# manasakani/DeviceKMC

Measured on AMD Instinct MI355X. Metric: KMC steps/sec, higher is better.
Workload: dtype f64

## Files before the change

### devicekmc_amd/csrc/common.h

```cpp
#pragma once
#include <hip/hip_runtime.h>
#include <stdint.h>
#include <stdio.h>
#include <string.h>
#include <math.h>
#include "../../include/devicekmc_hip.h"
#include "../../include/devicekmc_hip_debug.h"

enum { DEFECT = 0, OXYGEN_DEFECT = 1, VACANCY = 2, O_EL = 3, Hf_EL = 4, Ni_EL = 5, Ti_EL = 6, Pt_EL = 7, N_EL = 8, NULL_ELEMENT = 9 };
enum { EV_GEN = 0, EV_REC = 1, EV_VDIFF = 2, EV_IDIFF = 3, EV_NULL = 4 };

#define DKMC_KB 8.617333262e-5
#define DKMC_Q 1.60217663e-19
#define DKMC_HBAR 1.054571817e-34
#define DKMC_MAX_LAYERS 5
#define WAVE 64

struct MetalSet { int n; const int *e; };

__device__ __forceinline__ bool is_metal(int el, const MetalSet &ms)
{
    bool r = false;
    for (int t = 0; t < ms.n; ++t) r |= (ms.e[t] == el);
    return r;
// ... 152 lines not shown
    int x_poly1_degree = 0;
    int x_poly_form_used = 0, x_poly_products = 0;
    int x_slab_poly = 0;
    int x_aux_warm = 0;
    int x_items_kc = 0;
    int x_apply_form = 0;
    int x_tile_f32 = 1;
    double x_tile_drop = 0.0;
    int x_tile_drop_unit = 0;
    int x_tile_drop_auto = 1;
    long long x_tile_drop_gate = 0;
    double x_tile_drop_used = 0.0;
    int xtl_census_form = 1;
    int x_static_tiles = 2;
    int x_static_gate = 0;
    int x_static_nM = -1;
    int x_static_verify = 0;
    int x_tile_f32_fail_once = 0;
    int x_nmul_form = 1;
    int x_nmul_lane_bytes = 16;
    int x_nmul_window = 2;
    int x_nmul_window_cap = 76 * 1024;
    int x_nmul_window_block = 320;
    int x_block = 16;
    int x_format = 1;
    int current_map = 0;
    int x_iter_hint = 0;
    int event_temperature = 0;
    int event_census = 0;
    int event_census_valid = 0;
    double event_census_info[16] = {0};
    dkmc_stats stats{};
    char err[512] = {0};
    int err_code = 0;
    double E_gen[DKMC_MAX_LAYERS] = {0}, E_rec[DKMC_MAX_LAYERS] = {0}, E_Vdiff[DKMC_MAX_LAYERS] = {0}, E_Odiff[DKMC_MAX_LAYERS] = {0};
    int num_layers = 0;
    static const int NBUF = 184;
    void *buf[NBUF] = {nullptr};
    size_t bufsz[NBUF] = {0};
};

constexpr int X_STATIC_GATE = 32768;
static inline int x_static_rule(int ns, int gate_override) { return ns >= (gate_override > 0 ? gate_override : X_STATIC_GATE) ? 1 : 0; }
Engine &eng();
int dkmc_fail(int code, const char *what, const char *file, int line);
void *scratch(int slot, size_t bytes);
// ... 66 lines not shown
```

### devicekmc_amd/csrc/engine.hip

```cpp
#include "common.h"
#include <stdlib.h>

int events_upload_layers();
void xstate_reset(const void *key);

static Engine g_engine;
Engine &eng() { return g_engine; }

int dkmc_fail(int code, const char *what, const char *file, int line)
{
    Engine &e = eng();
    snprintf(e.err, sizeof(e.err), "%s (%s:%d)", what, file, line);
    e.err_code = code ? code : -1;
    fprintf(stderr, "devicekmc_hip: %s\n", e.err);
    return e.err_code;
}

void *scratch(int slot, size_t bytes)
{
    Engine &e = eng();
    if (bytes == 0) bytes = 16;
    if (e.bufsz[slot] < bytes) {
        if (e.buf[slot]) { (void)hipStreamSynchronize(e.stream); (void)hipFree(e.buf[slot]); }
        size_t want = bytes + bytes / 8 + 256;
// ... 64 lines not shown
void dkmc_set_x_tile_drop_auto(int on) { eng().x_tile_drop_auto = on ? 1 : 0; }
int dkmc_get_x_tile_drop_auto(void) { return eng().x_tile_drop_auto; }
void dkmc_set_x_tile_drop_auto_subblocks(long long gate) { eng().x_tile_drop_gate = gate > 0 ? gate : 0; }
double dkmc_get_x_tile_drop_used(void) { return eng().x_tile_drop_used; }
void dkmc_debug_fail_true_residual_once(void) { eng().x_tile_f32_fail_once = 1; }
void dkmc_set_x_static_tiles(int mode) { eng().x_static_tiles = (mode == 0 || mode == 1) ? mode : 2; }
int dkmc_get_x_static_tiles(void) { return eng().x_static_tiles; }
int dkmc_debug_x_static_verify(int on) { const int was = eng().x_static_verify; eng().x_static_verify = on ? 1 : 0; return was; }
void dkmc_debug_set_x_static_gate(int members) { eng().x_static_gate = members > 0 ? members : 0; }
int dkmc_x_static_rule(int members) { return x_static_rule(members, eng().x_static_gate); }
int dkmc_x_static_strips(int n_metals) { return n_metals > 0 ? n_metals / 256 : 0; }
void dkmc_set_x_nmul_form(int form) { eng().x_nmul_form = form == 0 ? 0 : 1; }
int dkmc_get_x_nmul_form(void) { return eng().x_nmul_form; }
void dkmc_set_x_nmul_lane_bytes(int bytes) { eng().x_nmul_lane_bytes = bytes == 8 ? 8 : 16; }
int dkmc_get_x_nmul_lane_bytes(void) { return eng().x_nmul_lane_bytes; }
void dkmc_set_x_nmul_window(int mode) { eng().x_nmul_window = (mode == 0 || mode == 1) ? mode : 2; }
int dkmc_get_x_nmul_window(void) { return eng().x_nmul_window; }
void dkmc_debug_set_x_nmul_window(int cap_bytes, int block_rows)
{
    Engine &e = eng();
    e.x_nmul_window_cap = cap_bytes < 0 ? 76 * 1024 : (cap_bytes > 76 * 1024 ? 76 * 1024 : cap_bytes);
    e.x_nmul_window_block = (block_rows >= 16 && block_rows <= 1024 && block_rows % 16 == 0) ? block_rows : 320;
}
void dkmc_set_x_slab(int on) { eng().x_slab = on ? 1 : 0; }
int dkmc_get_x_slab(void) { return eng().x_slab; }
void dkmc_set_x_slab_poly(int on) { eng().x_slab_poly = on ? 1 : 0; }
int dkmc_get_x_slab_poly(void) { return eng().x_slab_poly; }
void dkmc_set_x_block(int s) { eng().x_block = s < 1 ? 1 : (s > 16 ? 16 : s); }
int dkmc_get_x_block(void) { return eng().x_block; }
void dkmc_set_x_aux(int mode) { eng().x_aux = mode < 0 ? 0 : (mode > 3 ? 2 : mode); }
int dkmc_get_x_aux(void) { return eng().x_aux; }
void dkmc_set_k_blocked(int on) { eng().k_blocked = on ? 1 : 0; }
int dkmc_get_k_blocked(void) { return eng().k_blocked; }
void dkmc_set_k_blocked_large(int on) { eng().k_blocked_large = on ? 1 : 0; }
int dkmc_get_k_blocked_large(void) { return eng().k_blocked_large; }
void dkmc_set_k_window_word_bytes(int bytes) { eng().k_window_word_bytes = bytes == 2 ? 2 : 4; }
int dkmc_get_k_window_word_bytes(void) { return eng().k_window_word_bytes; }
void dkmc_set_cb_edge_domain(int atoms_only) { eng().cb_edge_domain = atoms_only ? 1 : 0; }

int dkmc_get_gpu_info(char *gpu_string, int capacity, int dev)
{
    hipDeviceProp_t prop;
    HIPCHK(hipSetDevice(dev));
    HIPCHK(hipGetDeviceProperties(&prop, dev));
    snprintf(gpu_string, capacity, "%s", prop.name);
    return 0;
// ... 117 lines not shown
```

### devicekmc_amd/csrc/nwin_plan.h

```cpp
#pragma once

#ifdef __HIPCC__
#define NWIN_HD __host__ __device__
#else
#define NWIN_HD
#endif

#define NWIN_ROW_BYTES 128
#define NWIN_CAP_BYTES (76 * 1024)
#define NWIN_BLOCK 320
#define NWIN_BLOCK_MAX 1024

struct NwinWindow { int lo, n; };

NWIN_HD inline int nwin_cap_rows(int cap_bytes) { return cap_bytes > 0 ? cap_bytes / NWIN_ROW_BYTES : 0; }
NWIN_HD inline int nwin_block_rows(int B) { return (B >= 16 && B <= NWIN_BLOCK_MAX && B % 16 == 0) ? B : NWIN_BLOCK; }
NWIN_HD inline int nwin_blocks(int m, int B) { return m > 0 ? (m + B - 1) / B : 0; }
NWIN_HD inline NwinWindow nwin_window(int m, int B, int cap_rows, int b)
{
    const int r0 = b * B, r1 = r0 + B < m ? r0 + B : m;
    if (cap_rows <= 0 || r0 >= m) return {0, 0};
    if (cap_rows < B) return {r0, r1 - r0 < cap_rows ? r1 - r0 : cap_rows};
    const int h = (cap_rows - B) / 2, lo = r0 - h > 0 ? r0 - h : 0, hi = r1 + h < m ? r1 + h : m;
    return {lo, hi - lo};
}
NWIN_HD inline int nwin_code(int c, NwinWindow W) { const int rel = c - W.lo; return (unsigned)rel < (unsigned)W.n ? rel : ~c; }
NWIN_HD inline int nwin_lds_bytes(int m, int B, int cap_rows)
{
    int n = B + 2 * ((cap_rows - B) / 2);
    if (cap_rows < B) n = cap_rows;
    if (n > m) n = m;
    return (n > 1 ? n : 1) * NWIN_ROW_BYTES;
}
NWIN_HD inline bool nwin_use(int mode, int m, int gate_rows) { return mode == 1 || (mode == 2 && m >= gate_rows); }
```

### devicekmc_amd/csrc/xtb_precond.h

```cpp
#pragma once
#include "nwin_plan.h"
__device__ __forceinline__ int xtb_xcd_block(int nb, int b) { const int xq = nb >> 3, xr = nb & 7, xc = b & 7; return xc * xq + min(xc, xr) + (b >> 3); }
template <int U> __device__ __forceinline__ int xn_bc(int x) { return __builtin_amdgcn_update_dpp(0, x, 0x150 + U, 0xf, 0xf, false); }
template <int J> __device__ __forceinline__ int xn_bc2(int x) { return __builtin_amdgcn_update_dpp(__builtin_amdgcn_update_dpp(0, x, 0x150 + 2 * J, 0xf, 0x3, false), x, 0x151 + 2 * J, 0xf, 0xc, false); }
struct XnEntry { int c, wlo, whi; };
__device__ __forceinline__ XnEntry xn_entry(int c, double w) { return {c, __double2loint(w), __double2hiint(w)}; }
template <int U> __device__ __forceinline__ double xn_w(XnEntry e) { return __hiloint2double(xn_bc<U>(e.whi), xn_bc<U>(e.wlo)); }
template <int J> __device__ __forceinline__ double xn_w2(XnEntry e) { return __hiloint2double(xn_bc2<J>(e.whi), xn_bc2<J>(e.wlo)); }
template <bool MASKED, int U> __device__ __forceinline__ double xn_gather(const double *panel, int v, int c)
{
    const int cu = xn_bc<U>(c);
    return (!MASKED || cu >= 0) ? *reinterpret_cast<const double *>(reinterpret_cast<const char *>(panel) + ((unsigned)cu * (unsigned)(XB_SP * 8) + (unsigned)(v * 8))) : 0.0;
}
struct XnX4 { double x0, x1, x2, x3; };
template <bool MASKED, int U> __device__ __forceinline__ XnX4 xn_gather4(const double *panel, int v, int c)
{
    return {xn_gather<MASKED, U>(panel, v, c), xn_gather<MASKED, U + 1>(panel, v, c), xn_gather<MASKED, U + 2>(panel, v, c), xn_gather<MASKED, U + 3>(panel, v, c)};
}
template <int J> __device__ __forceinline__ double2 xn_gather2(const double *panel, int v8, int c)
{ return *reinterpret_cast<const double2 *>(reinterpret_cast<const char *>(panel) + ((unsigned)xn_bc2<J>(c) * (unsigned)(XB_SP * 8) + (unsigned)(v8 * 16))); }
struct XnSums { double s0, s1, s2, s3; };
template <int U> __device__ __forceinline__ XnSums xn_acc4(XnEntry e, XnX4 x, XnSums s)
{
    s.s0 += xn_w<U>(e) * x.x0; s.s1 += xn_w<U + 1>(e) * x.x1; s.s2 += xn_w<U + 2>(e) * x.x2; s.s3 += xn_w<U + 3>(e) * x.x3; return s;
// ... 19 lines not shown
    const int v = threadIdx.x & 15, g = threadIdx.x >> 4;
    const int li = xtb_xcd_block((int)gridDim.x, (int)blockIdx.x) * 16 + g;
    const bool ok = li < m;
    const int row = LIST ? (ok ? rowlist[li] : 0) : li;
    const bool atom = ok && row >= 2;
    const xrp_t p0 = atom ? rp[row] : 0, p1 = atom ? rp[row + 1] : 0;
    const double scr = ok ? sc[row] : 0.0;
    const double av = ok ? add[(size_t)row * XB_SP + v] : 0.0;
    XnSums s = {0.0, 0.0, 0.0, 0.0};
    for (xrp_t base = p0; base < p1; base += 64) {
        int cm[4]; double wm[4];
#pragma unroll
        for (int bq = 0; bq < 4; ++bq) { const xrp_t pe = base + 16 * bq + v; int c = pe < p1 ? ci[pe] : -1; if (c < 2 || c == row) c = -1; cm[bq] = c; wm[bq] = c >= 0 ? val[pe] : 0.0; }
#pragma unroll
        for (int bq = 0; bq < 4; ++bq) wm[bq] = cm[bq] >= 0 ? wm[bq] * sc[cm[bq]] : 0.0;
#pragma unroll
        for (int bq = 0; bq < 4; ++bq) {
            if (base + 16 * bq >= p1) break;
            s = xn_batch16(in, v, xn_entry(cm[bq], wm[bq]), s);
        }
    }
    if (ok) out[(size_t)row * XB_SP + v] = xn_result(ca, av, cb, scr, s);
}
__global__ void k_xtb_npack_width(int m, const xrp_t *__restrict__ rp, int *__restrict__ cnt, const int *__restrict__ rowlist = nullptr)
{
    const int q = blockIdx.x * blockDim.x + threadIdx.x;
    if (q >= (m + 3) / 4) return;
    int w = 0;
    for (int r = 0; r < 4; ++r) {
        const int li = 4 * q + r; if (li >= m) continue;
        const int row = rowlist ? rowlist[li] : li;
        if (row >= 2) w = max(w, (int)(rp[row + 1] - rp[row]));
    }
    cnt[q] = 4 * w;
}
__global__ __launch_bounds__(256) void k_xtb_npack(int m, const xrp_t *__restrict__ rp, const int *__restrict__ ci, const double *__restrict__ val,
                                                   const double *__restrict__ sc, const long long *__restrict__ off, int *__restrict__ pcol, double *__restrict__ pw,
                                                   const int *__restrict__ rowlist = nullptr)
{
    const int q = blockIdx.x * 4 + (threadIdx.x >> 6), lane = threadIdx.x & 63;
    if (q >= (m + 3) / 4) return;
    const long long o0 = off[q], n = off[q + 1] - o0;
    for (long long i = lane; i < n; i += 64) {
        const int r = (int)(i & 3), k = (int)(i >> 2), li = 4 * q + r;
        const int row = rowlist ? rowlist[li < m ? li : m - 1] : li;
        const bool atom = row >= 2 && li < m;
        const xrp_t p0 = atom ? rp[row] : 0, len = atom ? rp[row + 1] - p0 : 0;
        int c = k < len ? ci[p0 + k] : -1;
        double w = 0.0;
// ... 131 lines not shown
            const int t = R.w - k0; const XnEntry e = xn_entry(nwin_code(n.c, W), n.w);
            if (t > 16) n = xn_slot(R, k0 + 16 + v);
            double2 x[4];
            x[0] = xn_operand2<0>(in, win, v8, e.c); x[1] = xn_operand2<1>(in, win, v8, e.c);
            if (t > 4) { x[2] = xn_operand2<2>(in, win, v8, e.c); x[3] = xn_operand2<3>(in, win, v8, e.c); }
            s = xn_acc2<0>(e, x[0], x[1], s);
            if (t > 4) s = xn_acc2<2>(e, x[2], x[3], s);
            if (t > 8) {
                x[0] = xn_operand2<4>(in, win, v8, e.c); x[1] = xn_operand2<5>(in, win, v8, e.c);
                if (t > 12) { x[2] = xn_operand2<6>(in, win, v8, e.c); x[3] = xn_operand2<7>(in, win, v8, e.c); }
                s = xn_acc2<4>(e, x[0], x[1], s);
                if (t > 12) s = xn_acc2<6>(e, x[2], x[3], s);
            }
        }
        if (QSF && wr) av = *reinterpret_cast<const double2 *>(add + (size_t)R.row * XB_SP + 2 * v8);
        const double tA0 = xor_lane<8>(s.A0), tA1 = xor_lane<8>(s.A1), tB0 = xor_lane<8>(s.B0), tB1 = xor_lane<8>(s.B1);
        if (wr) {
            const double o0 = xn_result(ca, av.x, cb, scr, {s.A0, tA0, s.B0, tB0}), o1 = xn_result(ca, av.y, cb, scr, {s.A1, tA1, s.B1, tB1});
            *reinterpret_cast<double2 *>(out + (size_t)R.row * XB_SP + 2 * v8) = make_double2(o0, o1);
            if (QSF) { const int sr = nsrank[R.row]; if (sr >= 0) { QS[xtb_qs_pos(sr, 2 * v8)] = scr * o0; QS[xtb_qs_pos(sr, 2 * v8 + 1)] = scr * o1; } }
        }
    }
}
__global__ void k_xtb_qs_from(int m, const double *__restrict__ V, const double *__restrict__ sc, const int *__restrict__ nsrank, double *__restrict__ QS, const XCtrl *ctrl)
{
    const int i = blockIdx.x * blockDim.x + threadIdx.x;
    if (i >= m * XB_SP || ctrl->done) return;
    const int row = i >> 4, v = i & 15;
    const int sr = nsrank[row];
    if (sr >= 0) QS[xtb_qs_pos(sr, v)] = sc[row] * V[i];
}
__global__ void k_xtb_pre_resid(int m, const double *__restrict__ T, const double *__restrict__ b, double *__restrict__ W)
{
    const int i = blockIdx.x * blockDim.x + threadIdx.x;
    if (i >= m * XB_SP) return;
    W[i] = (i & 15) == 0 ? T[i] - b[i >> 4] : 0.0;
}
__global__ void k_xtb_pre_col0(int m, const double *__restrict__ y, double *__restrict__ W)
{
    const int i = blockIdx.x * blockDim.x + threadIdx.x;
    if (i >= m * XB_SP) return;
    W[i] = (i & 15) == 0 ? y[i >> 4] : 0.0;
}
__global__ void k_xtb_pre_add(int m, const double *__restrict__ Z, double *__restrict__ y)
{
    const int i = blockIdx.x * blockDim.x + threadIdx.x;
// ... 3 lines not shown
__device__ __forceinline__ double xtb_tree256(double a)
{
    __shared__ double red[256];
    red[threadIdx.x] = a;
    __syncthreads();
    for (int o = 128; o > 0; o >>= 1) { if ((int)threadIdx.x < o) red[threadIdx.x] += red[threadIdx.x + o]; __syncthreads(); }
    return red[0];
}
__global__ __launch_bounds__(256) void k_xtb_pre_rr_part(int m, const double *__restrict__ T, const double *__restrict__ b, double *__restrict__ part)
{
    double a = 0.0;
    for (int i = blockIdx.x * 256 + threadIdx.x; i < m; i += gridDim.x * 256) { const double d = T[(size_t)i * XB_SP] - b[i]; a += d * d; }
    a = xtb_tree256(a);
    if (threadIdx.x == 0) part[blockIdx.x] = a;
}
__global__ __launch_bounds__(256) void k_xtb_pre_rr(int np, const double *__restrict__ part, double *__restrict__ out)
{
    double a = 0.0;
    for (int i = threadIdx.x; i < np; i += 256) a += part[i];
    a = xtb_tree256(a);
    if (threadIdx.x == 0) out[0] = a;
}

struct XbNPack { const long long *off; const int *col; const double *w; int lane_bytes; int win_B, win_rows; };
static const int xb_nwin_rows = 450000;
template <class Alloc>
static int xtb_npack(const XtbArgs &A, int n, const int *rowlist, Alloc alloc, long long pad, XbNPack *np)
{
    Engine &e = eng(); hipStream_t st = e.stream;
    const int nsl = (n + 3) / 4;
    int *cnt = (int *)alloc(S_XTB_NPACK_CNT, (size_t)nsl * 4);
    long long *off = (long long *)alloc(S_XTB_NPACK_OFF, (size_t)(nsl + 1) * 8);
    if (!cnt || !off) return e.err_code;
    hipLaunchKernelGGL(k_xtb_npack_width, dim3((nsl + 255) / 256), dim3(256), 0, st, n, A.rp, cnt, rowlist);
    if (int rc = dkmc_exclusive_scan_i32_i64(cnt, off, nsl, off + nsl)) return rc;
    long long nslot = 0;
    HIPCHK(hipMemcpyAsync(&nslot, off + nsl, sizeof(long long), hipMemcpyDeviceToHost, st));
    HIPCHK(hipStreamSynchronize(st));
    int *col = (int *)alloc(S_XTB_NPACK_COL, (size_t)(nslot + pad) * 4);
    double *w = (double *)alloc(S_XTB_NPACK_W, (size_t)(nslot + pad) * 8);
    if (!col || !w) return e.err_code;
    hipLaunchKernelGGL(k_xtb_npack, dim3((nsl + 3) / 4), dim3(256), 0, st, n, A.rp, A.ci, A.val, A.sc, (const long long *)off, col, w, rowlist);
    KCHK();
    np->off = off; np->col = col; np->w = w; np->lane_bytes = e.x_nmul_lane_bytes;
    const bool win = !rowlist && np->lane_bytes == 16 && nwin_use(e.x_nmul_window, n, xb_nwin_rows);
    np->win_B = win ? nwin_block_rows(e.x_nmul_window_block) : 0;
    np->win_rows = win ? nwin_cap_rows(std::min(std::max(e.x_nmul_window_cap, 0), NWIN_CAP_BYTES)) : 0;
    return 0;
}
struct XbNRank { int n; const int *rowlist; const XbNPack *np; double *QS; const XCtrl *ctrl; };
template <bool LIST>
static void xtb_nstep(hipStream_t st, const XtbArgs &A, const XbNRank &R, const double *in, const double *add, double ca, double cb, double *out, bool qsf)
{
    const dim3 g((R.n + 15) / 16), b(XT_NT);
    if (!R.np) { hipLaunchKernelGGL(k_xtb_nmul<LIST>, g, b, 0, st, R.n, A.rp, A.ci, A.val, A.sc, in, add, ca, cb, out, R.ctrl, R.rowlist); return; }
    if (!LIST && R.np->win_B > 0) {
        const int B = R.np->win_B, lds = nwin_lds_bytes(R.n, B, R.np->win_rows);
        const auto kw = qsf ? k_xtb_nmulw<true> : k_xtb_nmulw<false>;
        static bool big_lds = false;
        if (!big_lds) {
            (void)hipFuncSetAttribute((const void *)k_xtb_nmulw<true>, hipFuncAttributeMaxDynamicSharedMemorySize, NWIN_CAP_BYTES);
            (void)hipFuncSetAttribute((const void *)k_xtb_nmulw<false>, hipFuncAttributeMaxDynamicSharedMemorySize, NWIN_CAP_BYTES);
            big_lds = true;
        }
        hipLaunchKernelGGL(kw, dim3(nwin_blocks(R.n, B)), dim3(XN_WIN_NT), lds, st, R.n, R.np->off, R.np->col, R.np->w, A.sc, in, add, ca, cb, out, R.ctrl,
                           qsf ? A.nsrank : (const int *)nullptr, qsf ? R.QS : (double *)nullptr, B, R.np->win_rows);
        return;
    }
    const bool b16 = R.np->lane_bytes == 16;
    const auto k = qsf ? (b16 ? k_xtb_nmulp16<true, LIST> : k_xtb_nmulp<true, LIST>) : (b16 ? k_xtb_nmulp16<false, LIST> : k_xtb_nmulp<false, LIST>);
    hipLaunchKernelGGL(k, g, b, 0, st, R.n, R.np->off, R.np->col, R.np->w, A.sc, in, add, ca, cb, out, R.ctrl, qsf ? A.nsrank : (const int *)nullptr,
                       qsf ? R.QS : (double *)nullptr, R.rowlist);
}
template <class Pn, class Pre, class Ranks>
static int xtb_applyL(hipStream_t st, const XtbArgs &A, int pd, const double *pc, Pn src, Pn dst, Pn w1, Pn w2, bool qs, Pre pre, Ranks ranks)
{
    Pn in = src;
    for (int i = 0; i < pd; ++i) {
// ... 77 lines not shown
}

extern "C" int dkmc_xtb_poly_coeffs(int degree, double *pc)
{
    if (degree < 1 || degree > XB_MAXPOLY || !pc) return dkmc_fail(13, "xtb_poly_coeffs: degree outside 1 ... 16", __FILE__, __LINE__);
    xtb_poly_coeffs(degree, pc);
    return 0;
}
extern "C" int dkmc_xtb_poly1_coeffs(int n, double *pc, double *qmin)
{
    if (n < 1 || n > XB_MAXPOLY1 || !pc) return dkmc_fail(13, "xtb_poly1_coeffs: degree outside 1 ... 20", __FILE__, __LINE__);
    xtb_poly1_coeffs(n, pc, qmin);
    return 0;
}
extern "C" int dkmc_xtb_poly_rule(int m) { return xtb_poly_rule(m, eng().x_poly_rows); }
__global__ void k_xtb_test_qs_decode(int ns, const double *__restrict__ QS, double *__restrict__ out)
{
    const int i = blockIdx.x * blockDim.x + threadIdx.x;
    if (i < ns * XB_SP) out[i] = QS[xtb_qs_pos(i >> 4, i & 15)];
}
static void *xtb_test_alloc(int slot, size_t bytes)
{
    return scratch(slot == S_XTB_NPACK_CNT ? S_XTB_TEST_NPCNT : slot == S_XTB_NPACK_OFF ? S_XTB_TEST_NPOFF : slot == S_XTB_NPACK_COL ? S_XTB_TEST_NPCOL : S_XTB_TEST_NPW, bytes);
}
static int xtb_test_qs_out(hipStream_t st, int ns, const double *QS, double *qs)
{
    double *dq = (double *)scratch(S_XTB_TEST_ADD, (size_t)ns * XB_SP * 8);
    if (!dq) return eng().err_code;
    hipLaunchKernelGGL(k_xtb_test_qs_decode, dim3((unsigned)(((size_t)ns * XB_SP + 255) / 256)), dim3(256), 0, st, ns, QS, dq);
    KCHK();
    HIPCHK(hipMemcpyAsync(qs, dq, (size_t)ns * XB_SP * 8, hipMemcpyDeviceToHost, st));
    return 0;
}
extern "C" int dkmc_xtb_test_nstep(int m, const long long *rp, const int *ci, const double *val, const double *sc, const double *in, const double *add,
                                   double ca, double cb, int form, const int *rowlist, int nlist, const int *nsrank, int ns, double *out, double *qs)
{
    Engine &e = eng(); hipStream_t st = e.stream;
    if (m < 1 || !rp || !sc || !in || !add || !out || (form != 0 && form != 1)) return dkmc_fail(13, "xtb_test_nstep: bad arguments", __FILE__, __LINE__);
    const long long nnz = rp[m];
    if (rp[0] != 0 || nnz < 0 || nnz > 0x7fffffffll || (nnz > 0 && (!ci || !val))) return dkmc_fail(13, "xtb_test_nstep: bad row pointers", __FILE__, __LINE__);
    for (int i = 0; i < m; ++i) if (rp[i + 1] < rp[i]) return dkmc_fail(13, "xtb_test_nstep: bad row pointers", __FILE__, __LINE__);
    for (long long p = 0; p < nnz; ++p) if (ci[p] < 0 || ci[p] >= m) return dkmc_fail(13, "xtb_test_nstep: column outside the rows", __FILE__, __LINE__);
    if (rowlist) {
        if (nlist < 1 || nlist > m) return dkmc_fail(13, "xtb_test_nstep: bad row list", __FILE__, __LINE__);
        for (int i = 0; i < nlist; ++i) if (rowlist[i] < 0 || rowlist[i] >= m) return dkmc_fail(13, "xtb_test_nstep: bad row list", __FILE__, __LINE__);
    }
// ... 112 lines not shown
```

### devicekmc_amd/lib.py

```python
import ctypes as C
import os

_HERE = os.path.dirname(os.path.abspath(__file__))
LIB_PATH = os.path.join(_HERE, "libdevicekmc_hip.so")

c_int_p = C.POINTER(C.c_int)
c_dbl_p = C.POINTER(C.c_double)
vp = C.c_void_p


class dkmc_gpubuf(C.Structure):
    _PTRS = ["site_charge", "site_power", "site_potential_boundary", "site_potential_charge", "site_temperature",
             "site_CB_edge", "T_bg", "atom_power", "atom_CB_edge", "atom_virtual_potentials", "atom_charge",
             "site_element", "atom_element", "site_x", "site_y", "site_z", "atom_x", "atom_y", "atom_z",
             "metal_types", "sigma", "k", "lattice", "freq", "neigh_idx", "site_layer",
             "Device_row_ptr_d", "Device_col_indices_d", "contact_left_row_ptr", "contact_left_col_indices",
             "contact_right_row_ptr", "contact_right_col_indices"]
    _INTS = ["Device_nnz", "contact_left_nnz", "contact_right_nnz", "num_metal_types_", "N_", "nn_", "N_atom_"]
    _fields_ = [(n, vp) for n in _PTRS] + [(n, C.c_int) for n in _INTS]


class dkmc_stats(C.Structure):
    _fields_ = [("cg_iters_K", C.c_int), ("cg_iters_CB", C.c_int), ("cg_iters_X", C.c_int),
                ("cg_rr_K", C.c_double), ("cg_rr_CB", C.c_double), ("cg_rr_X", C.c_double),
# ... 57 lines not shown
    "dkmc_get_x_tile_drop_auto": (_I, []),
    "dkmc_get_x_tile_drop_used": (_D, []),
    "dkmc_get_x_tile_live_info": (_I, [C.POINTER(C.c_longlong), c_dbl_p]),
    "dkmc_xt_get_live": (_I, [_D, vp, vp]),
    "dkmc_xt_get_live_masks": (_I, [_D, vp]),
    "dkmc_debug_fail_true_residual_once": (None, []),
    "dkmc_set_x_static_tiles": (None, [_I]),
    "dkmc_get_x_static_tiles": (_I, []),
    "dkmc_get_x_static_info": (_I, [C.POINTER(C.c_longlong)]),
    "dkmc_debug_x_static_verify": (_I, [_I]),
    "dkmc_debug_get_x_static_verify": (_I, [C.POINTER(C.c_longlong)]),
    "dkmc_x_static_strips": (_I, [_I]),
    "dkmc_x_static_rule": (_I, [_I]),
    "dkmc_debug_set_x_static_gate": (None, [_I]),
    "dkmc_xt_get_srow": (_I, [c_int_p, vp]),
    "dkmc_xt_get_diag": (_I, [vp]),
    "dkmc_set_x_nmul_form": (None, [_I]),
    "dkmc_get_x_nmul_form": (_I, []),
    "dkmc_set_x_nmul_lane_bytes": (None, [_I]),
    "dkmc_get_x_nmul_lane_bytes": (_I, []),
    "dkmc_set_x_nmul_window": (None, [_I]),
    "dkmc_get_x_nmul_window": (_I, []),
    "dkmc_debug_set_x_nmul_window": (None, [_I, _I]),
    "dkmc_set_x_apply_form": (None, [_I]),
    "dkmc_get_x_apply_form": (_I, []),
    "dkmc_set_x_slab": (None, [_I]),
    "dkmc_get_x_slab": (_I, []),
    "dkmc_set_x_slab_poly": (None, [_I]),
    "dkmc_get_x_slab_poly": (_I, []),
    "dkmc_set_x_aux_warm": (None, [_I]),
    "dkmc_get_x_aux_warm": (_I, []),
    "dkmc_set_x_aux": (None, [_I]),
    "dkmc_get_x_aux": (_I, []),
    "dkmc_set_k_blocked": (None, [_I]),
    "dkmc_get_k_blocked": (_I, []),
    "dkmc_set_k_blocked_large": (None, [_I]),
    "dkmc_get_k_blocked_large": (_I, []),
    "dkmc_set_k_window_word_bytes": (None, [_I]),
    "dkmc_get_k_window_word_bytes": (_I, []),
    "dkmc_kcg_form_info": (_I, [C.POINTER(dkmc_gpubuf), C.POINTER(C.c_longlong)]),
    "dkmc_kcg_form_words": (_I, [C.POINTER(dkmc_gpubuf), C.POINTER(C.c_longlong)]),
    "dkmc_debug_kbw_halfword_pos": (_I, [_I, _I]),
    "dkmc_debug_kbw_segment_cap": (None, [_I]),
    "dkmc_set_pair_cutoff": (None, [_D]),
    "dkmc_reset_pair_sum_cache": (None, []),
    "dkmc_set_pair_form": (None, [_I]),
# ... 162 lines not shown
```

### include/devicekmc_hip.h

```cpp
#ifndef DEVICEKMC_HIP_H
#define DEVICEKMC_HIP_H

#ifdef __cplusplus
extern "C" {
#endif

#ifndef DKMC_ELEMENT_T
#define DKMC_ELEMENT_T int
#endif
typedef struct dkmc_gpubuf {
    int *site_charge;
    double *site_power, *site_potential_boundary, *site_potential_charge, *site_temperature;
    double *site_CB_edge;
    double *T_bg;
    double *atom_power;
    double *atom_CB_edge;
    double *atom_virtual_potentials;
    int *atom_charge;
    DKMC_ELEMENT_T *site_element;
    DKMC_ELEMENT_T *atom_element;
    double *site_x, *site_y, *site_z;
    double *atom_x, *atom_y, *atom_z;
    DKMC_ELEMENT_T *metal_types;
    double *sigma, *k, *lattice, *freq;
// ... 66 lines not shown
int dkmc_get_x_poly_auto(void);
void dkmc_set_x_poly_form(int form);
int dkmc_get_x_poly_form(void);
int dkmc_get_x_poly_form_used(void);
int dkmc_get_x_poly_products(void);
void dkmc_set_x_nmul_form(int form);
int dkmc_get_x_nmul_form(void);
void dkmc_set_x_tile_f32(int mode);
int dkmc_get_x_tile_f32(void);
void dkmc_set_x_tile_drop(double theta);
double dkmc_get_x_tile_drop(void);
void dkmc_set_x_tile_drop_unit(int unit);
int dkmc_get_x_tile_drop_unit(void);
void dkmc_set_x_tile_drop_auto(int on);
int dkmc_get_x_tile_drop_auto(void);
double dkmc_get_x_tile_drop_used(void);
void dkmc_set_x_static_tiles(int mode);
int dkmc_get_x_static_tiles(void);
int dkmc_get_x_static_info(long long *info8);
void dkmc_set_x_nmul_lane_bytes(int bytes);
int dkmc_get_x_nmul_lane_bytes(void);
void dkmc_set_x_nmul_window(int mode);
int dkmc_get_x_nmul_window(void);
void dkmc_set_x_slab(int on);
int dkmc_get_x_slab(void);
void dkmc_set_x_slab_poly(int on);
int dkmc_get_x_slab_poly(void);
void dkmc_set_k_slab(int on);
int dkmc_get_k_slab(void);
void dkmc_set_x_aux(int mode);
int dkmc_get_x_aux(void);
void dkmc_set_x_aux_warm(int on);
int dkmc_get_x_aux_warm(void);
void dkmc_set_k_blocked(int on);
int dkmc_get_k_blocked(void);
void dkmc_set_k_blocked_large(int on);
int dkmc_get_k_blocked_large(void);
void dkmc_set_k_window_word_bytes(int bytes);
int dkmc_get_k_window_word_bytes(void);
void dkmc_set_current_warm_start(int mode);
int dkmc_get_current_warm_start(void);
int dkmc_get_current_warm_vector(const dkmc_gpubuf *buf, double *h_out, int capacity, int *n_out);
int dkmc_set_current_warm_vector(const dkmc_gpubuf *buf, const double *h_in, int n);
int dkmc_get_current_warm_aux(const dkmc_gpubuf *buf, double *h_out, long long capacity, long long *n_out);
int dkmc_set_current_warm_aux(const dkmc_gpubuf *buf, const double *h_in, long long n);
void dkmc_set_profiling(int on);
// ... 168 lines not shown
```

### include/devicekmc_hip_debug.h

```cpp
#ifndef DEVICEKMC_HIP_DEBUG_H
#define DEVICEKMC_HIP_DEBUG_H
#include "devicekmc_hip.h"
#ifdef __cplusplus
extern "C" {
#endif

int dkmc_xt_time_share(int nranks, int rank, int reps, double *apply_us, double *side_us , int *items_out, long long *subblocks_out);
int dkmc_xt_check_shares(int nranks, double *max_abs_diff, double *max_abs, long long *subblocks_sum, long long *items_sum, int *items_total);
int dkmc_xtb_check_product(int width, double *max_abs_diff, double *max_abs);
int dkmc_xtb_poly_coeffs(int degree, double *pc);
int dkmc_xtb_poly_rule(int m);
void dkmc_set_x_poly_auto_rows(int n0, int n1);
int dkmc_xtb_test_nstep(int m, const long long *rp, const int *ci, const double *val, const double *sc, const double *in, const double *add,
                        double ca, double cb, int form, const int *rowlist, int nlist, const int *nsrank, int ns, double *out, double *qs);
int dkmc_xtb_check_poly(int degree, int form, const double *in, double *out, double *qs);
void dkmc_debug_set_x_nmul_window(int cap_bytes, int block_rows);
int dkmc_xtb_time_poly(int degree, int reps, double *us);
typedef struct dkmc_xtb_ctrl { double rr[2]; int done_local, sharded; int done; int iters; int abort_local, aborted; int pad[2]; int xchg_timeout, pad2; } dkmc_xtb_ctrl;
int dkmc_xtb_test_gram(int m, const double *P, const double *T, const double *R, const int *nsrank, int ns, int ng, int done_word, double *gfin,
                       dkmc_xtb_ctrl *ctrl_out);
int dkmc_xtb_test_small(int it, int s, int nrg, const double *gblocks, double tol2, const dkmc_xtb_ctrl *ctrl_in, double *mats, dkmc_xtb_ctrl *ctrl_out);
int dkmc_xtb_test_step(int m, int it, const double *mats, int done_word, double *y0, double *R, double *P, const double *T, const double *sc,
                       const int *nsrank, int ns, const int *rowlist, int nlist, double *Ypanel, double *qs);
int dkmc_xtb_poly1_coeffs(int n, double *pc, double *qmin);
void dkmc_debug_set_x_poly1_degree(int n);
int dkmc_xtb_test_gram1(int m, const double *const *panels, int ng, int done_word, double *gfin);
int dkmc_xtb_test_step1(int m, int it, const double *mats, int done_word, double *y0, double *const *panels, const double *sc, const int *nsrank, int ns,
                        double *qs);
int dkmc_xtb_time_apply(int width, int variant, int reps, double *us);
int dkmc_xt_tile_census(long long *hist);
void dkmc_set_x_items(int kc);
void dkmc_debug_fail_true_residual_once(void);
int dkmc_xtb_tile_product(int width, int stored_bytes, double *out);
int dkmc_xt_get_tiles(long long *ntiles, long long *nsub, int *tiles4, double *tval);
int dkmc_xtb_time_apply_stored(int width, int stored_bytes, int reps, double *us);
int dkmc_get_x_tile_live_info(long long *info8, double *ms2);
int dkmc_debug_xtl_census_form(int form);
long long dkmc_debug_xtl_census_reread(void);
double dkmc_xtl_drop_rule(long long stored_subblocks);
// ... 47 lines not shown
```

Before: 5.266.

## Add class-coded packed neighbor multiply that drops the per-slot weight array

```diff
diff --git a/devicekmc_amd/csrc/common.h b/devicekmc_amd/csrc/common.h
--- a/devicekmc_amd/csrc/common.h
+++ b/devicekmc_amd/csrc/common.h
@@ -198,6 +198,11 @@
     int x_nmul_window = 2;
     int x_nmul_window_cap = 76 * 1024;
     int x_nmul_window_block = 320;
+    int x_nmul_coded = 2;
+    int x_nmul_coded_cap = 76 * 1024;
+    int x_nmul_coded_block = 320;
+    int x_nmul_coded_halo = 126;
+    int x_nmul_coded_list = 0;
     int x_block = 16;
     int x_format = 1;
     int current_map = 0;
diff --git a/devicekmc_amd/csrc/engine.hip b/devicekmc_amd/csrc/engine.hip
--- a/devicekmc_amd/csrc/engine.hip
+++ b/devicekmc_amd/csrc/engine.hip
@@ -110,6 +110,16 @@
     e.x_nmul_window_cap = cap_bytes < 0 ? 76 * 1024 : (cap_bytes > 76 * 1024 ? 76 * 1024 : cap_bytes);
     e.x_nmul_window_block = (block_rows >= 16 && block_rows <= 1024 && block_rows % 16 == 0) ? block_rows : 320;
 }
+void dkmc_set_x_nmul_coded(int mode) { eng().x_nmul_coded = (mode == 0 || mode == 1) ? mode : 2; }
+int dkmc_get_x_nmul_coded(void) { return eng().x_nmul_coded; }
+void dkmc_debug_set_x_nmul_lists(int cap_bytes, int block_rows, int halo_rows, int list_rows)
+{
+    Engine &e = eng();
+    e.x_nmul_coded_cap = cap_bytes < 0 ? 76 * 1024 : (cap_bytes > 76 * 1024 ? 76 * 1024 : cap_bytes);
+    e.x_nmul_coded_block = (block_rows >= 16 && block_rows <= 1024 && block_rows % 16 == 0) ? block_rows : 320;
+    e.x_nmul_coded_halo = (halo_rows >= 0 && halo_rows <= 4096) ? halo_rows : 126;
+    e.x_nmul_coded_list = 0; (void)list_rows;
+}
 void dkmc_set_x_slab(int on) { eng().x_slab = on ? 1 : 0; }
 int dkmc_get_x_slab(void) { return eng().x_slab; }
 void dkmc_set_x_slab_poly(int on) { eng().x_slab_poly = on ? 1 : 0; }
diff --git a/devicekmc_amd/csrc/nwin_plan.h b/devicekmc_amd/csrc/nwin_plan.h
--- a/devicekmc_amd/csrc/nwin_plan.h
+++ b/devicekmc_amd/csrc/nwin_plan.h
@@ -33,3 +33,25 @@
     return (n > 1 ? n : 1) * NWIN_ROW_BYTES;
 }
 NWIN_HD inline bool nwin_use(int mode, int m, int gate_rows) { return mode == 1 || (mode == 2 && m >= gate_rows); }
+
+#define NWINC_ROW_BYTES (NWIN_ROW_BYTES + 8)
+#define NWINC_CLS_SHIFT 30
+#define NWINC_COL_MASK 0x3fffffffu
+#define NWINC_MAX_ROWS (1 << 28)
+#define NWINC_BLOCK 320
+#define NWINC_HALO 126
+#define NWINC_HALO_MAX 4096
+
+NWIN_HD inline unsigned nwinc_word(int c, int cls) { return (unsigned)c | ((unsigned)cls << NWINC_CLS_SHIFT); }
+NWIN_HD inline int nwinc_col(unsigned w) { return (int)(w & NWINC_COL_MASK); }
+NWIN_HD inline int nwinc_cls(unsigned w) { return (int)(w >> NWINC_CLS_SHIFT); }
+NWIN_HD inline int nwinc_block_rows(int B) { return (B >= 16 && B <= NWIN_BLOCK_MAX && B % 16 == 0) ? B : NWINC_BLOCK; }
+NWIN_HD inline int nwinc_halo_rows(int h) { return (h >= 0 && h <= NWINC_HALO_MAX) ? h : NWINC_HALO; }
+NWIN_HD inline int nwinc_rows(int cap_bytes, int B, int halo_rows)
+{
+    const int n = cap_bytes > 0 ? cap_bytes / NWINC_ROW_BYTES : 0;
+    return n > B + 2 * halo_rows ? B + 2 * halo_rows : n;
+}
+NWIN_HD inline int nwinc_lds_bytes(int m, int B, int win_rows) { return nwin_lds_bytes(m, B, win_rows) / NWIN_ROW_BYTES * NWINC_ROW_BYTES; }
+NWIN_HD inline bool nwinc_far(unsigned w, NwinWindow W) { return nwinc_cls(w) != 0 && nwin_code(nwinc_col(w), W) < 0; }
+NWIN_HD inline bool nwinc_use(int mode, int m, int gate_rows) { return m < NWINC_MAX_ROWS && (mode == 1 || (mode == 2 && m >= gate_rows)); }
diff --git a/devicekmc_amd/csrc/xtb_precond.h b/devicekmc_amd/csrc/xtb_precond.h
--- a/devicekmc_amd/csrc/xtb_precond.h
+++ b/devicekmc_amd/csrc/xtb_precond.h
@@ -65,9 +65,10 @@
     }
     if (ok) out[(size_t)row * XB_SP + v] = xn_result(ca, av, cb, scr, s);
 }
-__global__ void k_xtb_npack_width(int m, const xrp_t *__restrict__ rp, int *__restrict__ cnt, const int *__restrict__ rowlist = nullptr)
+__global__ void k_xtb_npack_width(int m, const xrp_t *__restrict__ rp, int *__restrict__ cnt, const int *__restrict__ rowlist = nullptr, unsigned long long *tab = nullptr)
 {
     const int q = blockIdx.x * blockDim.x + threadIdx.x;
+    if (tab && q < 4) tab[q] = 0;
     if (q >= (m + 3) / 4) return;
     int w = 0;
     for (int r = 0; r < 4; ++r) {
@@ -245,6 +246,133 @@
         }
     }
 }
+__device__ __forceinline__ unsigned long long xn_readlane64(unsigned long long x, int l)
+{ return ((unsigned long long)(unsigned)__builtin_amdgcn_readlane((int)(x >> 32), l) << 32) | (unsigned)__builtin_amdgcn_readlane((int)x, l); }
+__global__ __launch_bounds__(256) void k_xtb_nclasses(int m, const xrp_t *__restrict__ rp, const int *__restrict__ ci, const double *__restrict__ val, unsigned long long *tab)
+{
+    const int q = blockIdx.x * 4 + (threadIdx.x >> 6), lane = threadIdx.x & 63;
+    if (q >= (m + 3) / 4 || __hip_atomic_load(tab + 3, __ATOMIC_RELAXED, __HIP_MEMORY_SCOPE_AGENT) != 0) return;
+    unsigned long long k[3];
+    for (int j = 0; j < 3; ++j) k[j] = __hip_atomic_load(tab + j, __ATOMIC_RELAXED, __HIP_MEMORY_SCOPE_AGENT);
+    bool over = false;
+    for (int r = 0; r < 4 && !over; ++r) {
+        const int row = 4 * q + r; if (row < 2 || row >= m) continue;
+        const xrp_t p1 = rp[row + 1];
+        for (xrp_t base = rp[row]; base < p1 && !over; base += 64) {
+            const xrp_t p = base + lane;
+            const int c = p < p1 ? ci[p] : -1;
+            const bool inN = c >= 2 && c != row;
+            const unsigned long long b = inN ? (unsigned long long)__double_as_longlong(val[p]) : 0ull;
+            if (__ballot(inN && (b << 1) == 0) != 0) { over = true; break; }
+            bool pend = inN && b != k[0] && b != k[1] && b != k[2];
+            for (unsigned long long mask = __ballot(pend); mask != 0 && !over; mask = __ballot(pend)) {
+                const int lead = __ffsll((long long)mask) - 1;
+                const unsigned long long bl = xn_readlane64(b, lead);
+                if (lane == lead) {
+                    bool found = false;
+                    for (int j = 0; j < 3 && !found; ++j) {
+                        if (k[j] == 0) k[j] = __hip_atomic_load(tab + j, __ATOMIC_RELAXED, __HIP_MEMORY_SCOPE_AGENT);
+                        if (k[j] == 0) { const unsigned long long o = atomicCAS(tab + j, 0ull, bl); k[j] = o == 0 ? bl : o; }
+                        found = k[j] == bl;
+                    }
+                }
+                for (int j = 0; j < 3; ++j) k[j] = xn_readlane64(k[j], lead);
+                over = bl != k[0] && bl != k[1] && bl != k[2];
+                pend = pend && b != bl;
+            }
+        }
+    }
+    if (over && lane == 0) __hip_atomic_store(tab + 3, 1ull, __ATOMIC_RELAXED, __HIP_MEMORY_SCOPE_AGENT);
+}
+__global__ __launch_bounds__(256) void k_xtb_npackc(int m, const xrp_t *__restrict__ rp, const int *__restrict__ ci, const double *__restrict__ val,
+                                                    const long long *__restrict__ off, unsigned *__restrict__ pcw, unsigned long long gb0, unsigned long long gb1,
+                                                    int B, int win_rows, int *__restrict__ farcnt)
+{
+    const int q = blockIdx.x * 4 + (threadIdx.x >> 6), lane = threadIdx.x & 63;
+    if (q >= (m + 3) / 4) return;
+    const NwinWindow W = nwin_window(m, B, win_rows, 4 * q / B);
+    const long long o0 = off[q], n = off[q + 1] - o0;
+    int far = 0;
+    for (long long i = lane; i < n; i += 64) {
+        const int r = (int)(i & 3), k = (int)(i >> 2), row = 4 * q + r;
+        const bool atom = row >= 2 && row < m;
+        const xrp_t p0 = atom ? rp[row] : 0, len = atom ? rp[row + 1] - p0 : 0;
+        int c = k < len ? ci[p0 + k] : -1, cls = 0;
+        if (c < 2 || c == row) c = row < m ? row : m - 1;
+        else { const unsigned long long b = (unsigned long long)__double_as_longlong(val[p0 + k]); cls = b == gb0 ? 1 : (b == gb1 ? 2 : 3); }
+        const unsigned w = nwinc_word(c, cls);
+        pcw[o0 + i] = w;
+        far += nwinc_far(w, W) ? 1 : 0;
+    }
+    for (int o = 32; o > 0; o >>= 1) far += __shfl_down(far, o);
+    if (lane == 0) farcnt[q] = far;
+}
+typedef const __attribute__((address_space(3))) double *xn_ldsd_t;
+template <bool QSF>
+__global__ __launch_bounds__(XN_WIN_NT) __attribute__((amdgpu_waves_per_eu(8, 8))) void k_xtb_nmulc(int m, const long long *__restrict__ off, const unsigned *__restrict__ pcw,
+                                                         const double *__restrict__ sc, const double *__restrict__ in, const double *__restrict__ add,
+                                                         double ca, double cb, double *__restrict__ out, const XCtrl *ctrl, const int *__restrict__ nsrank, double *__restrict__ QS,
+                                                         int B, int win_rows, double g1, double g2, double g3)
+{
+    extern __shared__ double2 xn_win[];
+    __shared__ long long xn_boff[NWIN_BLOCK_MAX / 4 + 1];
+    if (ctrl->done) return;
+    const int blk = xtb_xcd_block((int)gridDim.x, (int)blockIdx.x);
+    const NwinWindow W = nwin_window(m, B, win_rows, blk);
+    const int q0 = blk * (B / 4), nq = min(B / 4, (m + 3) / 4 - q0);
+    for (int i = threadIdx.x; i <= nq; i += XN_WIN_NT) xn_boff[i] = off[q0 + i];
+    {
+        const double2 *src = reinterpret_cast<const double2 *>(in + (size_t)W.lo * XB_SP);
+        const int n16 = W.n * 8;
+#pragma unroll 4
+        for (int i = threadIdx.x; i < n16; i += XN_WIN_NT) xn_win[i] = src[i];
+        double *scd = reinterpret_cast<double *>(xn_win + n16);
+        for (int i = threadIdx.x; i < W.n; i += XN_WIN_NT) scd[i] = sc[W.lo + i];
+    }
+    __syncthreads();
+    const xn_lds_t win = (xn_lds_t)xn_win;
+    const xn_ldsd_t scw = (xn_ldsd_t)(win + (unsigned)W.n * (unsigned)NWIN_ROW_BYTES);
+    const int v = threadIdx.x & 15, r = (threadIdx.x >> 4) & 3, v8 = v & 7;
+    for (int sl = __builtin_amdgcn_readfirstlane(threadIdx.x >> 6); sl < nq; sl += XN_WIN_NT / 64) {
+        const long long o0 = xn_boff[sl]; const int w = (int)((xn_boff[sl + 1] - o0) >> 2);
+        const unsigned *cq = pcw + o0 + r;
+        unsigned nw = v < w ? cq[4 * v] : 0u;
+        const int row = 4 * (q0 + sl) + r;
+        const bool ok = row < m, wr = ok && v < 8;
+        const int rcode = nwin_code(row, W);
+        double scr = scw[max(rcode, 0)];
+        if (rcode < 0) scr = ok ? sc[row] : 0.0;
+        double2 av = (!QSF && wr) ? *reinterpret_cast<const double2 *>(add + (size_t)row * XB_SP + 2 * v8) : make_double2(0.0, 0.0);
+        XnSums2 s = {0.0, 0.0, 0.0, 0.0};
+        for (int k0 = 0; k0 < w; k0 += 16) {
+            const int t = w - k0; const unsigned cw = nw;
+            if (t > 16) nw = k0 + 16 + v < w ? cq[4 * (k0 + 16 + v)] : 0u;
+            const int col = nwinc_col(cw), cls = nwinc_cls(cw), code = nwin_code(col, W);
+            double scv = scw[max(code, 0)];
+            if (code < 0 && cls != 0) scv = sc[col];
+            const double gv = cls == 1 ? g1 : (cls == 2 ? g2 : g3);
+            const XnEntry e = xn_entry(code, cls != 0 ? gv * scv : 0.0);
+            double2 x[4];
+            x[0] = xn_operand2<0>(in, win, v8, e.c); x[1] = xn_operand2<1>(in, win, v8, e.c);
+            if (t > 4) { x[2] = xn_operand2<2>(in, win, v8, e.c); x[3] = xn_operand2<3>(in, win, v8, e.c); }
+            s = xn_acc2<0>(e, x[0], x[1], s);
+            if (t > 4) s = xn_acc2<2>(e, x[2], x[3], s);
+            if (t > 8) {
+                x[0] = xn_operand2<4>(in, win, v8, e.c); x[1] = xn_operand2<5>(in, win, v8, e.c);
+                if (t > 12) { x[2] = xn_operand2<6>(in, win, v8, e.c); x[3] = xn_operand2<7>(in, win, v8, e.c); }
+                s = xn_acc2<4>(e, x[0], x[1], s);
+                if (t > 12) s = xn_acc2<6>(e, x[2], x[3], s);
+            }
+        }
+        if (QSF && wr) av = *reinterpret_cast<const double2 *>(add + (size_t)row * XB_SP + 2 * v8);
+        const double tA0 = xor_lane<8>(s.A0), tA1 = xor_lane<8>(s.A1), tB0 = xor_lane<8>(s.B0), tB1 = xor_lane<8>(s.B1);
+        if (wr) {
+            const double o0v = xn_result(ca, av.x, cb, scr, {s.A0, tA0, s.B0, tB0}), o1v = xn_result(ca, av.y, cb, scr, {s.A1, tA1, s.B1, tB1});
+            *reinterpret_cast<double2 *>(out + (size_t)row * XB_SP + 2 * v8) = make_double2(o0v, o1v);
+            if (QSF) { const int sr = nsrank[row]; if (sr >= 0) { QS[xtb_qs_pos(sr, 2 * v8)] = scr * o0v; QS[xtb_qs_pos(sr, 2 * v8 + 1)] = scr * o1v; } }
+        }
+    }
+}
 __global__ void k_xtb_qs_from(int m, const double *__restrict__ V, const double *__restrict__ sc, const int *__restrict__ nsrank, double *__restrict__ QS, const XCtrl *ctrl)
 {
     const int i = blockIdx.x * blockDim.x + threadIdx.x;
@@ -294,30 +422,61 @@
     if (threadIdx.x == 0) out[0] = a;
 }
 
-struct XbNPack { const long long *off; const int *col; const double *w; int lane_bytes; int win_B, win_rows; };
+struct XbNPack { const long long *off; const int *col; const double *w; int lane_bytes; int win_B, win_rows; int coded; double g[3]; };
 static const int xb_nwin_rows = 450000;
+static const int xb_ncoded_rows = 450000;
+struct XbNInfo { long long form = 0, classes = -1, slots = 0, lds = 0; const int *dfar = nullptr; int nsl = 0; hipEvent_t e0 = nullptr, e1 = nullptr; bool timed = false; };
+static XbNInfo g_xn_info;
+static bool xtb_ninfo_events(XbNInfo &I)
+{
+    if (!I.e0 && (hipEventCreate(&I.e0) != hipSuccess || hipEventCreate(&I.e1) != hipSuccess)) { I.e0 = I.e1 = nullptr; (void)hipGetLastError(); }
+    return I.e0 != nullptr;
+}
 template <class Alloc>
 static int xtb_npack(const XtbArgs &A, int n, const int *rowlist, Alloc alloc, long long pad, XbNPack *np)
 {
     Engine &e = eng(); hipStream_t st = e.stream;
     const int nsl = (n + 3) / 4;
+    XbNInfo &I = g_xn_info;
+    const bool timed = !rowlist && xtb_ninfo_events(I);
+    if (timed) HIPCHK(hipEventRecord(I.e0, st));
     int *cnt = (int *)alloc(S_XTB_NPACK_CNT, (size_t)nsl * 4);
-    long long *off = (long long *)alloc(S_XTB_NPACK_OFF, (size_t)(nsl + 1) * 8);
+    long long *off = (long long *)alloc(S_XTB_NPACK_OFF, (size_t)(nsl + 1 + 4) * 8);
     if (!cnt || !off) return e.err_code;
-    hipLaunchKernelGGL(k_xtb_npack_width, dim3((nsl + 255) / 256), dim3(256), 0, st, n, A.rp, cnt, rowlist);
+    const bool win = !rowlist && e.x_nmul_lane_bytes == 16 && nwin_use(e.x_nmul_window, n, xb_nwin_rows);
+    const bool try_coded = win && nwinc_use(e.x_nmul_coded, n, xb_ncoded_rows);
+    unsigned long long *tab = try_coded ? (unsigned long long *)(off + nsl + 1) : nullptr;
+    hipLaunchKernelGGL(k_xtb_npack_width, dim3((nsl + 255) / 256), dim3(256), 0, st, n, A.rp, cnt, rowlist, tab);
+    if (try_coded) hipLaunchKernelGGL(k_xtb_nclasses, dim3((nsl + 3) / 4), dim3(256), 0, st, n, A.rp, A.ci, A.val, tab);
     if (int rc = dkmc_exclusive_scan_i32_i64(cnt, off, nsl, off + nsl)) return rc;
-    long long nslot = 0;
-    HIPCHK(hipMemcpyAsync(&nslot, off + nsl, sizeof(long long), hipMemcpyDeviceToHost, st));
+    unsigned long long back[5] = {0, 0, 0, 0, 0};
+    HIPCHK(hipMemcpyAsync(back, off + nsl, try_coded ? sizeof(back) : sizeof(long long), hipMemcpyDeviceToHost, st));
     HIPCHK(hipStreamSynchronize(st));
+    const long long nslot = (long long)back[0];
+    const unsigned long long *tabh = back + 1;
+    const bool coded = try_coded && tabh[3] == 0;
     int *col = (int *)alloc(S_XTB_NPACK_COL, (size_t)(nslot + pad) * 4);
-    double *w = (double *)alloc(S_XTB_NPACK_W, (size_t)(nslot + pad) * 8);
-    if (!col || !w) return e.err_code;
-    hipLaunchKernelGGL(k_xtb_npack, dim3((nsl + 3) / 4), dim3(256), 0, st, n, A.rp, A.ci, A.val, A.sc, (const long long *)off, col, w, rowlist);
+    double *w = coded ? nullptr : (double *)alloc(S_XTB_NPACK_W, (size_t)(nslot + pad) * 8);
+    if (!col || (!coded && !w)) return e.err_code;
+    np->off = off; np->col = col; np->w = w; np->lane_bytes = e.x_nmul_lane_bytes; np->coded = coded ? 1 : 0;
+    if (coded) {
+        np->win_B = nwinc_block_rows(e.x_nmul_coded_block);
+        np->win_rows = nwinc_rows(std::min(std::max(e.x_nmul_coded_cap, 0), NWIN_CAP_BYTES), np->win_B, nwinc_halo_rows(e.x_nmul_coded_halo));
+        for (int j = 0; j < 3; ++j) memcpy(&np->g[j], &tabh[j], 8);
+        hipLaunchKernelGGL(k_xtb_npackc, dim3((nsl + 3) / 4), dim3(256), 0, st, n, A.rp, A.ci, A.val, (const long long *)off, (unsigned *)col, tabh[0], tabh[1],
+                           np->win_B, np->win_rows, cnt);
+    } else {
+        np->win_B = win ? nwin_block_rows(e.x_nmul_window_block) : 0;
+        np->win_rows = win ? nwin_cap_rows(std::min(std::max(e.x_nmul_window_cap, 0), NWIN_CAP_BYTES)) : 0;
+        hipLaunchKernelGGL(k_xtb_npack, dim3((nsl + 3) / 4), dim3(256), 0, st, n, A.rp, A.ci, A.val, A.sc, (const long long *)off, col, w, rowlist);
+    }
     KCHK();
-    np->off = off; np->col = col; np->w = w; np->lane_bytes = e.x_nmul_lane_bytes;
-    const bool win = !rowlist && np->lane_bytes == 16 && nwin_use(e.x_nmul_window, n, xb_nwin_rows);
-    np->win_B = win ? nwin_block_rows(e.x_nmul_window_block) : 0;
-    np->win_rows = win ? nwin_cap_rows(std::min(std::max(e.x_nmul_window_cap, 0), NWIN_CAP_BYTES)) : 0;
+    if (!rowlist) {
+        if (timed) HIPCHK(hipEventRecord(I.e1, st));
+        I.timed = timed; I.form = coded ? 1 : 0; I.slots = nslot; I.dfar = coded ? cnt : nullptr; I.nsl = nsl;
+        I.classes = !try_coded ? -1 : (tabh[3] != 0 ? 4 : (tabh[0] != 0) + (tabh[1] != 0) + (tabh[2] != 0));
+        I.lds = coded ? nwinc_lds_bytes(n, np->win_B, np->win_rows) : (win ? nwin_lds_bytes(n, np->win_B, np->win_rows) : 0);
+    }
     return 0;
 }
 struct XbNRank { int n; const int *rowlist; const XbNPack *np; double *QS; const XCtrl *ctrl; };
@@ -326,6 +485,19 @@
 {
     const dim3 g((R.n + 15) / 16), b(XT_NT);
     if (!R.np) { hipLaunchKernelGGL(k_xtb_nmul<LIST>, g, b, 0, st, R.n, A.rp, A.ci, A.val, A.sc, in, add, ca, cb, out, R.ctrl, R.rowlist); return; }
+    if (!LIST && R.np->coded) {
+        const int B = R.np->win_B, lds = nwinc_lds_bytes(R.n, B, R.np->win_rows);
+        const auto kc = qsf ? k_xtb_nmulc<true> : k_xtb_nmulc<false>;
+        static bool big_lds = false;
+        if (!big_lds) {
+            (void)hipFuncSetAttribute((const void *)k_xtb_nmulc<true>, hipFuncAttributeMaxDynamicSharedMemorySize, NWIN_CAP_BYTES);
+            (void)hipFuncSetAttribute((const void *)k_xtb_nmulc<false>, hipFuncAttributeMaxDynamicSharedMemorySize, NWIN_CAP_BYTES);
+            big_lds = true;
+        }
+        hipLaunchKernelGGL(kc, dim3(nwin_blocks(R.n, B)), dim3(XN_WIN_NT), lds, st, R.n, R.np->off, (const unsigned *)R.np->col, A.sc, in, add, ca, cb, out, R.ctrl,
+                           qsf ? A.nsrank : (const int *)nullptr, qsf ? R.QS : (double *)nullptr, B, R.np->win_rows, R.np->g[0], R.np->g[1], R.np->g[2]);
+        return;
+    }
     if (!LIST && R.np->win_B > 0) {
         const int B = R.np->win_B, lds = nwin_lds_bytes(R.n, B, R.np->win_rows);
         const auto kw = qsf ? k_xtb_nmulw<true> : k_xtb_nmulw<false>;
@@ -449,6 +621,21 @@
 static void *xtb_test_alloc(int slot, size_t bytes)
 {
     return scratch(slot == S_XTB_NPACK_CNT ? S_XTB_TEST_NPCNT : slot == S_XTB_NPACK_OFF ? S_XTB_TEST_NPOFF : slot == S_XTB_NPACK_COL ? S_XTB_TEST_NPCOL : S_XTB_TEST_NPW, bytes);
+}
+extern "C" int dkmc_get_x_nmul_coded_info(long long info[8])
+{
+    Engine &e = eng(); const XbNInfo &I = g_xn_info;
+    if (!info) return dkmc_fail(13, "get_x_nmul_coded_info: null", __FILE__, __LINE__);
+    long long far = -1, us = -1;
+    if (I.form == 1 && I.dfar) {
+        std::vector<int> f((size_t)I.nsl);
+        HIPCHK(hipMemcpyAsync(f.data(), I.dfar, (size_t)I.nsl * 4, hipMemcpyDeviceToHost, e.stream));
+        HIPCHK(hipStreamSynchronize(e.stream));
+        far = 0; for (int x : f) far += x;
+    }
+    if (I.timed) { float ms = 0.f; HIPCHK(hipEventSynchronize(I.e1)); HIPCHK(hipEventElapsedTime(&ms, I.e0, I.e1)); us = (long long)(ms * 1e3f + 0.5f); }
+    info[0] = I.form; info[1] = I.classes; info[2] = I.slots; info[3] = far; info[4] = 0; info[5] = far; info[6] = I.lds; info[7] = us;
+    return e.err_code;
 }
 static int xtb_test_qs_out(hipStream_t st, int ns, const double *QS, double *qs)
 {
diff --git a/devicekmc_amd/lib.py b/devicekmc_amd/lib.py
--- a/devicekmc_amd/lib.py
+++ b/devicekmc_amd/lib.py
@@ -103,6 +103,10 @@
     "dkmc_set_x_nmul_window": (None, [_I]),
     "dkmc_get_x_nmul_window": (_I, []),
     "dkmc_debug_set_x_nmul_window": (None, [_I, _I]),
+    "dkmc_set_x_nmul_coded": (None, [_I]),
+    "dkmc_get_x_nmul_coded": (_I, []),
+    "dkmc_get_x_nmul_coded_info": (_I, [C.POINTER(C.c_longlong)]),
+    "dkmc_debug_set_x_nmul_lists": (None, [_I, _I, _I, _I]),
     "dkmc_set_x_apply_form": (None, [_I]),
     "dkmc_get_x_apply_form": (_I, []),
     "dkmc_set_x_slab": (None, [_I]),
diff --git a/include/devicekmc_hip.h b/include/devicekmc_hip.h
--- a/include/devicekmc_hip.h
+++ b/include/devicekmc_hip.h
@@ -112,6 +112,9 @@
 int dkmc_get_x_nmul_lane_bytes(void);
 void dkmc_set_x_nmul_window(int mode);
 int dkmc_get_x_nmul_window(void);
+void dkmc_set_x_nmul_coded(int mode);
+int dkmc_get_x_nmul_coded(void);
+int dkmc_get_x_nmul_coded_info(long long info[8]);
 void dkmc_set_x_slab(int on);
 int dkmc_get_x_slab(void);
 void dkmc_set_x_slab_poly(int on);
diff --git a/include/devicekmc_hip_debug.h b/include/devicekmc_hip_debug.h
--- a/include/devicekmc_hip_debug.h
+++ b/include/devicekmc_hip_debug.h
@@ -15,6 +15,7 @@
                         double ca, double cb, int form, const int *rowlist, int nlist, const int *nsrank, int ns, double *out, double *qs);
 int dkmc_xtb_check_poly(int degree, int form, const double *in, double *out, double *qs);
 void dkmc_debug_set_x_nmul_window(int cap_bytes, int block_rows);
+void dkmc_debug_set_x_nmul_lists(int cap_bytes, int block_rows, int halo_rows, int list_rows);
 int dkmc_xtb_time_poly(int degree, int reps, double *us);
 typedef struct dkmc_xtb_ctrl { double rr[2]; int done_local, sharded; int done; int iters; int abort_local, aborted; int pad[2]; int xchg_timeout, pad2; } dkmc_xtb_ctrl;
 int dkmc_xtb_test_gram(int m, const double *P, const double *T, const double *R, const int *nsrank, int ns, int ng, int done_word, double *gfin,
```

Result: faster. 5.377, median of 6 (+2.1%).
